# TorchIO-project/torchio

Hardware: NVIDIA H100
Metric: augmented voxels/sec on 256^3 fp32 Compose pipeline (higher is better)
Workload: dtype f32

## Files before the change

include/tio_b200.h:

```cpp
#ifndef TIO_B200_H
#define TIO_B200_H

#include <stddef.h>
#include <stdint.h>

#ifdef __cplusplus
extern "C" {
#endif

#define TIO_ABI_VERSION 2

enum tio_dtype {
  TIO_F32 = 0,
  TIO_U8 = 1,
  TIO_I8 = 2,
  TIO_I16 = 3,
  TIO_I32 = 4,
  TIO_I64 = 5,
  TIO_F16 = 6,
  TIO_BF16 = 7,
  TIO_F64 = 8
};

enum tio_interp { TIO_NEAREST = 0, TIO_LINEAR = 1, TIO_LABEL_PV = 2 };
#define TIO_EXACT_COORDS 0x100

#define TIO_FLAG_PASSTHROUGH 1u
#define TIO_FLAG_ELASTIC 2u

const char* tio_last_error(void);
int tio_abi_version(void);
uint64_t tio_launch_count(void);

size_t tio_resample_workspace_bytes(int B, int OI, int OJ, int OK);

int tio_bspline_prefilter(const void* src, int dtype, float* coeff, const uint8_t* flags,
                          int B, int C, int I, int J, int K, int order, void* stream);
int tio_bspline_resample(const float* coeff, const void* src, void* dst, int dtype,
                         int B, int C, int I, int J, int K,
                         int OI, int OJ, int OK,
                         const float* mat, const float* cp, const uint8_t* flags,
                         int ni, int nj, int nk,
                         const float* spacing_in, const float* spacing_out,
                         int affine_first, int order, void* stream);
int tio_resample(const void* src, void* dst, int dtype,
                 int B, int C, int I, int J, int K,
                 int OI, int OJ, int OK,
                 const float* mat, const float* cp, const uint8_t* flags,
                 int ni, int nj, int nk,
                 const float* spacing_in, const float* spacing_out,
                 int affine_first, int mode, const float* fill, int box_hint,
                 void* workspace, size_t workspace_bytes, void* stream);

int tio_onehot(const void* src, int dtype, int B, int64_t vox, const void* labels, int n,
               float* dst, void* stream);
int tio_label_argmax(const float* sampled, int B, int n, int64_t vox, const void* labels,
                     float pad_label, void* dst, int dtype, void* stream);

int tio_crop_patches(const void* src, void* dst, int elem_bytes, int C, int I, int J, int K,
                     int n, const int32_t* corners, int pi, int pj, int pk, void* stream);

int tio_remap(const void* src, void* dst, int elem_bytes, int B, int C, int I, int J, int K,
              int OI, int OJ, int OK, int off_i, int off_j, int off_k, int mode,
              const void* fill, const uint8_t* flip, void* stream);

int tio_permute(const void* src, void* dst, int elem_bytes, int B, int C, int I, int J, int K,
                int perm0, int perm1, int perm2, int flip_bits, void* stream);

int tio_upload(const void* host_pinned, void* dst_device, size_t bytes, void* stream);

int tio_min_sample0(const float* src, int C, int64_t n, float* fill, void* stream);

int tio_blur(const float* src, float* dst, float* scratch,
             int B, int C, int I, int J, int K,
             const float* taps, const int32_t* radius, int R, int axes_mask,
             const uint8_t* identity, void* stream);

size_t tio_mt19937_table_bytes(void);
int tio_mt19937_build_table(void* host_blob, size_t bytes);
size_t tio_randn_mt19937_workspace_bytes(uint64_t offset, uint64_t n);
int tio_randn_mt19937(uint64_t seed, uint64_t offset, uint64_t n, float* z,
                      const void* table, void* workspace, size_t workspace_bytes,
                      void* stream);

int tio_moments(const float* src, const uint8_t* mask, int64_t n, double* out3, void* stream);
// ... 113 lines not shown
```

torchio_b200/csrc/resample.cu:

```cuda
#include "resample_common.cuh"

namespace tio {

template <typename T, int MODE, bool HAS_CP, bool HAS_FILL>
__global__ void __launch_bounds__(TK* TJ)
resample_kernel(const ResampleArgs a) {
  extern __shared__ float smem_cp[];
  const int tiles_i = (a.OI + TI - 1) / TI;
  const int b = blockIdx.z / tiles_i;
  const int oi0 = (blockIdx.z % tiles_i) * TI;
  const int ok = blockIdx.x * TK + threadIdx.x;
  const int oj = blockIdx.y * TJ + threadIdx.y;
  const int64_t n_in = (int64_t)a.I * a.J * a.K;
  const int64_t n_out = (int64_t)a.OI * a.OJ * a.OK;
  const uint8_t fl = a.flags ? a.flags[b] : 0;
  const T* __restrict__ src = (const T*)a.src + (int64_t)b * a.C * n_in;
  T* __restrict__ dst = (T*)a.dst + (int64_t)b * a.C * n_out;
  const int oi_end = min(oi0 + TI, a.OI);

  if (fl & TIO_FLAG_PASSTHROUGH) {
    if (ok < a.OK && oj < a.OJ)
      for (int c = 0; c < a.C; ++c)
        for (int oi = oi0; oi < oi_end; ++oi) {
          int64_t o = ((int64_t)oi * a.OJ + oj) * a.OK + ok;
// ... 80 lines not shown
  int c = blockIdx.x * blockDim.x + threadIdx.x;
  if (c < C) fill[c] = __int_as_float(0x7f800000);
}

template <bool VEC>
__global__ void __launch_bounds__(256) min_kernel(const float* __restrict__ src, int64_t n,
                                                  float* fill) {
  const int c = blockIdx.y;
  const float* base = src + (int64_t)c * n;
  float m = __int_as_float(0x7f800000);
  const int64_t stride = (int64_t)gridDim.x * blockDim.x;
  const int64_t t0 = (int64_t)blockIdx.x * blockDim.x + threadIdx.x;
  if (VEC) {
    const float4* p = (const float4*)base;
    for (int64_t t = t0; t < (n >> 2); t += stride) {
      float4 v = __ldg(p + t);
      m = fminf(fminf(m, v.x), fminf(v.y, fminf(v.z, v.w)));
    }
  } else {
    for (int64_t t = t0; t < n; t += stride) m = fminf(m, __ldg(base + t));
  }
#pragma unroll
  for (int s = 16; s > 0; s >>= 1) m = fminf(m, __shfl_xor_sync(0xffffffffu, m, s));
  __shared__ float part[8];
  if ((threadIdx.x & 31) == 0) part[threadIdx.x >> 5] = m;
  __syncthreads();
  if (threadIdx.x == 0) {
    for (int t = 1; t < 8; ++t) m = fminf(m, part[t]);
    atomic_min_float(fill + c, m);
  }
}

int launch_resample_tile(const ResampleArgs& a, int dtype, int mode, bool exact_coords, int box_hint,
                         void* workspace, size_t workspace_bytes, cudaStream_t st);
size_t resample_tile_workspace_bytes(int B, int OI, int OJ, int OK);

}

extern "C" int tio_resample(const void* src, void* dst, int dtype, int B, int C, int I, int J,
                            int K, int OI, int OJ, int OK, const float* mat, const float* cp,
                            const uint8_t* flags, int ni, int nj, int nk,
                            const float* spacing_in, const float* spacing_out,
                            int affine_first, int mode, const float* fill, int box_hint,
                            void* workspace, size_t workspace_bytes, void* stream) {
  using namespace tio;
  TIO_CHECK_ARG(src && dst && mat, "tio_resample: null src/dst/mat");
  TIO_CHECK_ARG(src != dst, "tio_resample: src and dst must not alias");
  TIO_CHECK_ARG(B > 0 && C > 0 && I > 0 && J > 0 && K > 0 && OI > 0 && OJ > 0 && OK > 0,
                "tio_resample: non-positive shape");
  const bool exact_coords = (mode & TIO_EXACT_COORDS) != 0;
  mode &= ~TIO_EXACT_COORDS;
  TIO_CHECK_ARG(mode == TIO_NEAREST || mode == TIO_LINEAR || mode == TIO_LABEL_PV, "tio_resample: bad mode %d", mode);
  TIO_CHECK_ARG(mode != TIO_LABEL_PV || (C == 1 && fill),
                "tio_resample: TIO_LABEL_PV needs C == 1 and fill[0] = the pad label");
  TIO_CHECK_ARG(spacing_in && spacing_out, "tio_resample: null spacing");
  TIO_CHECK_ARG(!cp || (ni >= 2 && nj >= 2 && nk >= 2), "tio_resample: control grid < 2 per axis");
  TIO_CHECK_ARG((int64_t)B * ((OI + TI - 1) / TI) <= 65535 && (OJ + TJ - 1) / TJ <= 65535,
                "tio_resample: grid too large (B*ceil(OI/16) and ceil(OJ/4) must be <= 65535)");
  ResampleArgs a;
  a.src = src; a.dst = dst; a.mat = mat; a.cp = cp; a.flags = flags; a.fill = fill;
  a.B = B; a.C = C; a.I = I; a.J = J; a.K = K; a.OI = OI; a.OJ = OJ; a.OK = OK;
  a.ni = ni; a.nj = nj; a.nk = nk;
  auto scale = [](int n_in, int n_out) {
    if (n_in == n_out) return 1.0f;
    return n_out > 1 ? (float)(n_in - 1) / (float)(n_out - 1) : 0.0f;
  };
  a.sc_i = cp ? scale(ni, OI) : 0.f; a.sc_j = cp ? scale(nj, OJ) : 0.f; a.sc_k = cp ? scale(nk, OK) : 0.f;
  const int dims[3] = {I, J, K};
  for (int t = 0; t < 3; ++t) {
    a.sp_in[t] = spacing_in[t]; a.sp_out[t] = spacing_out[t];
    a.nm1[t] = (float)(dims[t] - 1 > 1 ? dims[t] - 1 : 1);
    a.sm1[t] = (float)(dims[t] - 1);
  }
  a.affine_first = affine_first;
  a.cp_in_smem = cp && ((size_t)ni * nj * nk * 12 <= 96 * 1024);
  cudaStream_t st = (cudaStream_t)stream;
  if (box_hint >= 0) {
    const int rc = launch_resample_tile(a, dtype, mode, exact_coords, box_hint, workspace, workspace_bytes, st);
    if (rc == 0) {
      TIO_CHECK_LAUNCH();
      return 0;
    }
    TIO_CHECK_ARG(rc == 1, "tio_resample: TMA tile path failed (code %d)", rc);
  }
  switch (dtype) {
    case TIO_F32: launch_typed<float>(a, mode, st); break;
    case TIO_U8: launch_typed<uint8_t>(a, mode, st); break;
    case TIO_I8: launch_typed<int8_t>(a, mode, st); break;
    case TIO_I16: launch_typed<int16_t>(a, mode, st); break;
    case TIO_I32: launch_typed<int32_t>(a, mode, st); break;
    case TIO_I64: launch_typed<int64_t>(a, mode, st); break;
    default: TIO_CHECK_ARG(false, "tio_resample: unknown dtype %d", dtype);
  }
  TIO_CHECK_LAUNCH();
  return 0;
}

extern "C" size_t tio_resample_workspace_bytes(int B, int OI, int OJ, int OK) {
  return tio::resample_tile_workspace_bytes(B, OI, OJ, OK);
}

extern "C" int tio_min_sample0(const float* src, int C, int64_t n, float* fill, void* stream) {
  using namespace tio;
  TIO_CHECK_ARG(src && fill && C > 0 && n > 0, "tio_min_sample0: bad arguments");
  cudaStream_t st = (cudaStream_t)stream;
  min_init_kernel<<<(C + 31) / 32, 32, 0, st>>>(fill, C);
  launched();
  const bool vec = (((uintptr_t)src & 15) == 0) && ((n & 3) == 0);
  int64_t work = vec ? (n >> 2) : n;
  int blocks = (int)((work + 255) / 256);
  if (blocks > num_sms() * 8) blocks = num_sms() * 8;
  if (blocks < 1) blocks = 1;
  if (vec)
    min_kernel<true><<<dim3(blocks, C), 256, 0, st>>>(src, n, fill);
  else
    min_kernel<false><<<dim3(blocks, C), 256, 0, st>>>(src, n, fill);
  launched();
  TIO_CHECK_LAUNCH();
  return 0;
}
```

torchio_b200/csrc/resample_common.cuh:

```cuda
#pragma once
#include "common.cuh"

namespace tio {


template <typename T>
struct ElemTraits;
template <>
struct ElemTraits<float> {
  static __device__ __forceinline__ float to_f32(float v) { return v; }
  static __device__ __forceinline__ float from_f32(float v) { return v; }
};
#define TIO_INT_TRAITS(T)                                                    \
  template <>                                                                \
  struct ElemTraits<T> {                                                     \
    static __device__ __forceinline__ float to_f32(T v) { return (float)v; } \
    static __device__ __forceinline__ T from_f32(float v) {                  \
      return (T)(long long)v;                \
    }                                                                        \
  };
TIO_INT_TRAITS(uint8_t)
TIO_INT_TRAITS(int8_t)
TIO_INT_TRAITS(int16_t)
TIO_INT_TRAITS(int32_t)
TIO_INT_TRAITS(int64_t)

struct ResampleArgs {
  const void* src;
  void* dst;
  const float* mat;
  const float* cp;
  const uint8_t* flags;
  const float* fill;
  int B, C, I, J, K, OI, OJ, OK;
  int ni, nj, nk;
  float sc_i, sc_j, sc_k;
  float sp_in[3], sp_out[3];
  float nm1[3];
  float sm1[3];
  int affine_first;
  int cp_in_smem;
};

constexpr int TK = 64;
constexpr int TJ = 4;
constexpr int TI = 16;

__device__ __forceinline__ float affine_row(const float* m, float pi, float pj, float pk) {
  float acc = __fmul_rn(pi, m[0]);
  acc = __fmaf_rn(pj, m[1], acc);
  acc = __fmaf_rn(pk, m[2], acc);
  acc = __fmaf_rn(1.0f, m[3], acc);
  return acc;
}

__device__ __forceinline__ float renormalise(float q, float nm1, float sm1) {
  float g = __fsub_rn(__fdiv_rn(__fmul_rn(2.0f, q), nm1), 1.0f);
  return __fmul_rn(__fmul_rn(__fadd_rn(g, 1.0f), 0.5f), sm1);
}


template <typename T>
__device__ __forceinline__ T label_pv_pick(const T tap[8], const float w[8], const unsigned active, const T pad) {
  if (active == 0u) return pad;
  {
    T first = tap[7];
// ... 206 lines not shown
```

torchio_b200/csrc/resample_fast.cu:

```cuda
#include <type_traits>

#include "resample_tile.cuh"

namespace tio {

template <int BOX, int LK>
__device__ __forceinline__ void lane_column(int tid, int& jrow, int& kcol) {
  const int warp = tid >> 5, lane = tid & 31;
  if (LK == 16) {
    constexpr int DJ = (BOX == 20) ? 2 : 4;
    const int half = lane >> 4;
    jrow = (warp % DJ) + (warp / DJ) * (2 * DJ) + half * DJ;
    kcol = lane & 15;
  } else if (LK == 8) {
    jrow = (warp >> 1) * 4 + (lane >> 3);
    kcol = (warp & 1) * 8 + (lane & 7);
  } else {
    jrow = (warp >> 2) * 8 + (lane >> 2);
    kcol = (warp & 3) * 4 + (lane & 3);
  }
}

template <bool HAS_CP, bool HAS_FILL>
__device__ __forceinline__ void exact_planes(const ResampleArgs& a, const TileArgs& ta, int b, bool elastic,
// ... 122 lines not shown
      unpack2(sub2(bc(tz[2 * ax + 1]), u[ax]), qa, qb);
      ma *= __saturatef(fminf(pa, qa));
      mb *= __saturatef(fminf(pb, qb));
    }
    if (!(ma > 0.5f)) va = fill_c;
    if (!(mb > 0.5f)) vb = fill_c;
    unc_a = fabsf(ma - 0.5f) < 1.0e-3f;
    unc_b = fabsf(mb - 0.5f) < 1.0e-3f;
  }
}

template <int BOX, bool HAS_CP, bool HAS_FILL>
__global__ void __launch_bounds__(256, BOX <= 22 ? 4 : 3)
resample_fast_kernel(const __grid_constant__ CUtensorMap tmap, const __grid_constant__ CUtensorMap tmap_s,
                     const __grid_constant__ ResampleArgs a, const __grid_constant__ TileArgs ta,
                     const int4* __restrict__ records) {
  constexpr int BK = box_k_extent(BOX, 4);
  constexpr int NBOX = BOX * BOX * BK;
  constexpr int BOXBYTES = (NBOX * 4 + 15) / 16 * 16;
  constexpr int C1 = BOX * BK, C2 = BK;
  constexpr bool DUAL = HAS_CP && BOX > kSmallBox;
  constexpr int BKS = box_k_extent(kSmallBox, 4);
  constexpr int NBOXS = kSmallBox * kSmallBox * BKS, C1S = kSmallBox * BKS, C2S = BKS;
  extern __shared__ __align__(128) unsigned char smem_raw[];
  float* aux = reinterpret_cast<float*>(smem_raw + BOXBYTES);
  const uint32_t box_u32 = smem_u32(smem_raw);
  const uint32_t bar = smem_u32(aux + 128);
  float* tbase = aux + 132;
  int* cell_tab = reinterpret_cast<int*>(aux + 136);
  unsigned* chg_mask = reinterpret_cast<unsigned*>(aux + 152);

  const int tid = threadIdx.x;
  const int tiles_i = ta.tiles_i;
  const int b = tiles_i == 1 ? (int)blockIdx.z : (int)__umulhi(blockIdx.z, ta.inv_tiles_i);
  const int ti = blockIdx.z - b * tiles_i;
  const int i0 = ti * XT, j0 = blockIdx.y * XT, k0 = blockIdx.x * XT;
  const unsigned tile_id = (blockIdx.z * gridDim.y + blockIdx.y) * gridDim.x + blockIdx.x;
  const int4 rec = __ldg(records + tile_id);
  if ((rec.w & (255 | 2048)) != (1 | 2048)) {
    slow_tile<HAS_CP, HAS_FILL>(a, ta, rec, b, i0, j0, k0);
    return;
  }
  const bool small = DUAL && (rec.w & 4096);
  if (tid == 0) {
    mbar_init(bar, 1);
    mbar_fence_init();
    mbar_expect_tx(bar, (uint32_t)((small ? NBOXS : NBOX) * 4));
    tma_load_4d(box_u32, small ? &tmap_s : &tmap, rec.z, rec.y, rec.x, b * a.C, bar);
  }
  const bool elastic = HAS_CP && (rec.w & 1024);
  const bool masked = HAS_FILL && !(rec.w & 256);
  const float* __restrict__ mp = a.mat + b * 12;
  if (tid >= 32 && tid < 35) {
    const int ax = tid - 32;
    const double t = (double)mp[4 * ax] * i0 + (double)mp[4 * ax + 1] * j0 + (double)mp[4 * ax + 2] * k0 +
                     (double)mp[4 * ax + 3] - (double)(ax == 0 ? rec.x : (ax == 1 ? rec.y : rec.z));
    tbase[ax] = (float)t;
  }
  if (HAS_CP && elastic && tid >= 64 && tid < 96) {
    const int lane = tid - 64;
    auto cell_of = [&](int rel) { return min((int)floorf(__fmul_rn(a.sc_i, (float)(i0 + rel))), a.ni - 1); };
    if (lane < XT) cell_tab[lane] = cell_of(lane);
    bool chg = false;
    if (lane < XT / 2)
      chg = lane == 0 || cell_of(2 * lane) != cell_of(2 * lane - 2) || cell_of(2 * lane + 1) != cell_of(2 * lane - 1);
    const unsigned mask = __ballot_sync(0xffffffffu, chg);
    if (lane == 0) *chg_mask = mask;
  }
// ... 206 lines not shown
```

torchio_b200/csrc/resample_tile.cu:

```cuda
#include <cuda.h>

#include <map>
#include <mutex>

#include "resample_tile.cuh"

namespace tio {

template <int BOX, typename T, int MODE, bool HAS_CP, bool CHECK, bool FASTDIV, int EMODE>
__device__ __forceinline__ void walk_column(
    const ResampleArgs& a, const TileArgs& ta, const T* __restrict__ box,
    const float* __restrict__ cps, const LiEntry* __restrict__ li_tab,
    const LiPair* __restrict__ li_pairs, const float m[12],
    const bool elastic, const bool identity, const uint32_t kbase, const int i0, const int i1,
    const int oj, const int ok, const float fill_c, T* __restrict__ out, const int64_t ostride) {
  constexpr int BK = box_k_extent(BOX, (int)sizeof(T));
  constexpr int C1 = BOX * BK, C2 = BK;
  constexpr int ESH = sizeof(T) == 1 ? 0 : (sizeof(T) == 2 ? 1 : 2);
  const float hd0 = ta.hd[0], hd1 = ta.hd[1], hd2 = ta.hd[2];
  const float rc0 = ta.rcp[0], rc1 = ta.rcp[1], rc2 = ta.rcp[2];
  const float hs0 = ta.hs[0], hs1 = ta.hs[1], hs2 = ta.hs[2];
  const float pj = (float)oj, pk = (float)ok;
  LerpAxis lj, lk;
  int o00 = 0, o01 = 0, o10 = 0, o11 = 0;
// ... 511 lines not shown
                          const TileArgs& ta, dim3 grid,
                          size_t smem, const int4* records, cudaStream_t st);

template <typename T>
static void launch_nearest(int box, const CUtensorMap& tm, const ResampleArgs& a, const TileArgs& ta,
                           dim3 grid, size_t smem, const int4* records, cudaStream_t st) {
  if (box == 24) {
    if (a.cp) launch_tile<24, T, TIO_NEAREST, true, true>(tm, a, ta, grid, smem, records, st);
    else launch_tile<24, T, TIO_NEAREST, false, true>(tm, a, ta, grid, smem, records, st);
  } else {
    if (a.cp) launch_tile<32, T, TIO_NEAREST, true, true>(tm, a, ta, grid, smem, records, st);
    else launch_tile<32, T, TIO_NEAREST, false, true>(tm, a, ta, grid, smem, records, st);
  }
}

template <typename T>
static void launch_label_pv(int box, const CUtensorMap& tm, const ResampleArgs& a, const TileArgs& ta,
                            dim3 grid, size_t smem, const int4* records, cudaStream_t st) {
  if (box == 24) {
    if (a.cp) launch_tile<24, T, TIO_LABEL_PV, true, true>(tm, a, ta, grid, smem, records, st);
    else launch_tile<24, T, TIO_LABEL_PV, false, true>(tm, a, ta, grid, smem, records, st);
  } else {
    if (a.cp) launch_tile<32, T, TIO_LABEL_PV, true, true>(tm, a, ta, grid, smem, records, st);
    else launch_tile<32, T, TIO_LABEL_PV, false, true>(tm, a, ta, grid, smem, records, st);
  }
}

size_t resample_tile_workspace_bytes(int B, int OI, int OJ, int OK) {
  const size_t tiles = (size_t)B * ((OI + XT - 1) / XT) * ((OJ + XT - 1) / XT) * ((OK + XT - 1) / XT);
  return tiles * sizeof(int4);
}

int launch_resample_tile(const ResampleArgs& a, int dtype, int mode, bool exact_coords, int box_hint,
                         void* workspace, size_t workspace_bytes, cudaStream_t st) {
  int esize = 0;
  if (mode == TIO_LINEAR) esize = dtype == TIO_F32 ? 4 : 0;
  else esize = dtype == TIO_U8 ? 1 : dtype == TIO_I16 ? 2 : dtype == TIO_I32 ? 4 : 0;
  if (!esize) return 1;
  const int kalign = 16 / esize;
  if (((int64_t)a.K * esize & 15) || ((uintptr_t)a.src & 15)) return 1;
  if ((int64_t)a.B * a.C > (1 << 30)) return 1;
  EncodeTiledFn encode = encode_tiled_fn();
  if (!encode) return 1;
  int box = 24;
  if (box_hint > 0) box = box_hint <= 20 ? 20 : box_hint <= 22 ? 22 : box_hint <= 24 ? 24 : box_hint <= 28 ? 28 : 32;
  if (mode != TIO_LINEAR) box = box <= 24 ? 24 : 32;
  const int tiles_i = (a.OI + XT - 1) / XT;
  if ((int64_t)a.B * tiles_i > 65535 || (a.OJ + XT - 1) / XT > 65535) return 1;

  CUtensorMap tm;
  const cuuint64_t gdim[4] = {(cuuint64_t)a.K, (cuuint64_t)a.J, (cuuint64_t)a.I, (cuuint64_t)a.B * a.C};
  const cuuint64_t gstride[3] = {(cuuint64_t)a.K * esize, (cuuint64_t)a.J * a.K * esize,
                                 (cuuint64_t)a.I * a.J * a.K * esize};
  const int bk = box_k_extent(box, esize);
  const cuuint32_t bdim[4] = {(cuuint32_t)bk, (cuuint32_t)box, (cuuint32_t)box, 1};
  const cuuint32_t estr[4] = {1, 1, 1, 1};
  const CUtensorMapDataType ttype = mode == TIO_LINEAR ? CU_TENSOR_MAP_DATA_TYPE_FLOAT32
                                    : esize == 1 ? CU_TENSOR_MAP_DATA_TYPE_UINT8
                                    : esize == 2 ? CU_TENSOR_MAP_DATA_TYPE_UINT16
                                                 : CU_TENSOR_MAP_DATA_TYPE_INT32;
  CUresult rc = encode(&tm, ttype, 4, const_cast<void*>(a.src), gdim, gstride,
                       bdim, estr, CU_TENSOR_MAP_INTERLEAVE_NONE, CU_TENSOR_MAP_SWIZZLE_NONE,
                       CU_TENSOR_MAP_L2_PROMOTION_L2_128B, CU_TENSOR_MAP_FLOAT_OOB_FILL_NONE);
  if (rc != CUDA_SUCCESS) return 1;

  TileArgs ta;
  const int dims[3] = {a.I, a.J, a.K};
  bool fast = true;
  for (int t = 0; t < 3; ++t) {
    ta.hd[t] = a.nm1[t] * 0.5f;
    ta.rcp[t] = (float)(1.0 / (double)ta.hd[t]);
    ta.hs[t] = a.sm1[t] * 0.5f;
    (void)dims;
    fast = fast && fastdiv_admitted(ta.hd[t], st);
  }
  ta.n_in = (long long)a.I * a.J * a.K;
  ta.n_out = (long long)a.OI * a.OJ * a.OK;
  ta.tiles_i = tiles_i;
  ta.inv_tiles_i = (unsigned)((1ull << 32) / (unsigned)tiles_i) + 1u;
  ta.sp_in_one = (a.sp_in[0] == 1.f && a.sp_in[1] == 1.f && a.sp_in[2] == 1.f);
  ta.sp_out_one = (a.sp_out[0] == 1.f && a.sp_out[1] == 1.f && a.sp_out[2] == 1.f);
  ta.magic_bytes = (unsigned)kMagicBits << 2;
  for (int t = 0; t < 3; ++t) {
    ta.rsp_in[t] = (float)(1.0 / (double)a.sp_in[t]);
    ta.rsp_out[t] = (float)(1.0 / (double)a.sp_out[t]);
  }

  dim3 grid((a.OK + XT - 1) / XT, (a.OJ + XT - 1) / XT, (unsigned)(a.B * tiles_i));
  const int64_t n_tiles = (int64_t)grid.x * grid.y * grid.z;
  if (n_tiles >= (1ll << 31)) return 1;
  if (!workspace || workspace_bytes < (size_t)n_tiles * sizeof(int4) || ((uintptr_t)workspace & 15)) return 1;
  int4* records = (int4*)workspace;
  const unsigned bounds_blocks = (unsigned)((n_tiles + 127) / 128);
  if (mode != TIO_LINEAR && !fast) return 1;
  const bool dual = !exact_coords && mode == TIO_LINEAR && a.cp && box > kSmallBox;
  const int box_s = dual ? kSmallBox : 0, bk_s = dual ? box_k_extent(kSmallBox, 4) : 0;
  CUtensorMap tm_small = tm;
  if (dual) {
    const cuuint32_t bdim_s[4] = {(cuuint32_t)bk_s, (cuuint32_t)box_s, (cuuint32_t)box_s, 1};
    if (encode(&tm_small, ttype, 4, const_cast<void*>(a.src), gdim, gstride, bdim_s, estr,
               CU_TENSOR_MAP_INTERLEAVE_NONE, CU_TENSOR_MAP_SWIZZLE_NONE, CU_TENSOR_MAP_L2_PROMOTION_L2_128B,
               CU_TENSOR_MAP_FLOAT_OOB_FILL_NONE) != CUDA_SUCCESS)
      return 1;
  }
  if (a.cp) tile_bounds_kernel<true><<<bounds_blocks, 128, 0, st>>>(a, box, kalign, bk, box_s, bk_s, records);
  else tile_bounds_kernel<false><<<bounds_blocks, 128, 0, st>>>(a, box, kalign, bk, box_s, bk_s, records);
  launched();
  const size_t smem = ((size_t)box * box * bk * esize + 15) / 16 * 16 + kAuxFloats * sizeof(float);
  if (mode == TIO_LABEL_PV) {
    if (dtype == TIO_U8) launch_label_pv<uint8_t>(box, tm, a, ta, grid, smem, records, st);
    else if (dtype == TIO_I16) launch_label_pv<int16_t>(box, tm, a, ta, grid, smem, records, st);
    else launch_label_pv<int32_t>(box, tm, a, ta, grid, smem, records, st);
    return 0;
  }
  if (mode == TIO_NEAREST) {
    if (dtype == TIO_U8) launch_nearest<uint8_t>(box, tm, a, ta, grid, smem, records, st);
    else if (dtype == TIO_I16) launch_nearest<int16_t>(box, tm, a, ta, grid, smem, records, st);
    else launch_nearest<int32_t>(box, tm, a, ta, grid, smem, records, st);
    return 0;
  }
  if (!exact_coords) {
    launch_resample_fast(box, tm, tm_small, a, ta, grid, smem, records, st);
    return 0;
  }
  if (box == 20) launch_box<20>(tm, a, ta, grid, smem, fast, records, st);
  else if (box == 22) launch_box<22>(tm, a, ta, grid, smem, fast, records, st);
  else if (box == 24) launch_box<24>(tm, a, ta, grid, smem, fast, records, st);
  else if (box == 28) launch_box<28>(tm, a, ta, grid, smem, fast, records, st);
  else launch_box<32>(tm, a, ta, grid, smem, fast, records, st);
  return 0;
}

}
```

torchio_b200/csrc/resample_tile.cuh:

```cuda
#pragma once
#include <cuda.h>

#include "resample_common.cuh"
#include "tma.cuh"

namespace tio {

constexpr int XT = 16;
constexpr int kSmallBox = 18;
__host__ __device__ constexpr int box_k_extent(int box, int elem_bytes) {
  return (box + 16 / elem_bytes + 16 / elem_bytes - 1) / (16 / elem_bytes) * (16 / elem_bytes);
}
constexpr float kMagic = 12582912.0f;
constexpr int kMagicBits = 0x4B400000;

struct TileArgs {
  float hd[3];
  float rcp[3];
  float hs[3];
  int sp_in_one, sp_out_one;
  float rsp_in[3], rsp_out[3];
  unsigned magic_bytes;
  long long n_in, n_out;
  int tiles_i;
// ... 53 lines not shown
    float b00 = lerp2(lk.l0, p1[o00 + ax], lk.l1, p1[o01 + ax]);
    float b01 = lerp2(lk.l0, p1[o10 + ax], lk.l1, p1[o11 + ax]);
    d[ax] = lerp2(li.l0, lerp2(lj.l0, a00, lj.l1, a01), li.l1, lerp2(lj.l0, b00, lj.l1, b01));
  }
}

__device__ __forceinline__ int axis_points(float scale, int lo, int hi, int* pts) {
  int n = 0;
  pts[n++] = lo;
  if (hi > lo) {
    const float rlo = scale * (float)lo, rhi = scale * (float)hi;
    const int c_first = (int)floorf(rlo) + 1, c_last = (int)ceilf(rhi) - 1;
    for (int c = c_first; c <= c_last; ++c) {
      if (n > 6) return -1;
      const int o = (int)floorf((float)c / scale);
      for (int t = o - 1; t <= o + 1; ++t)
        if (t > lo && t < hi && t > pts[n - 1]) pts[n++] = t;
    }
    pts[n++] = hi;
    if (n > 8) return -1;
  }
  return n;
}

template <bool HAS_CP>
__global__ void __launch_bounds__(128)
tile_bounds_kernel(const ResampleArgs a, const int box, const int kalign, const int bk, const int box_s,
                   const int bk_s, int4* __restrict__ records) {
  const int tiles_i = (a.OI + XT - 1) / XT, tiles_j = (a.OJ + XT - 1) / XT, tiles_k = (a.OK + XT - 1) / XT;
  const int64_t n_tiles = (int64_t)a.B * tiles_i * tiles_j * tiles_k;
  const int64_t tile = (int64_t)blockIdx.x * blockDim.x + threadIdx.x;
  if (tile >= n_tiles) return;
  const unsigned per_b = (unsigned)(tiles_i * tiles_j * tiles_k);
  const int b = (int)(tile / per_b);
  unsigned rest = (unsigned)(tile - (int64_t)b * per_b);
  const int tk = (int)(rest % (unsigned)tiles_k);
  rest /= (unsigned)tiles_k;
  const int tj = (int)(rest % (unsigned)tiles_j), ti = (int)(rest / (unsigned)tiles_j);
  const int i0 = ti * XT, j0 = tj * XT, k0 = tk * XT;
  const int i1 = min(i0 + XT, a.OI) - 1, j1 = min(j0 + XT, a.OJ) - 1, k1 = min(k0 + XT, a.OK) - 1;
  const uint8_t fl = a.flags ? a.flags[b] : 0;
  if (fl & TIO_FLAG_PASSTHROUGH) {
    records[tile] = make_int4(0, 0, 0, 3);
    return;
  }
  const bool elastic = HAS_CP && (fl & TIO_FLAG_ELASTIC);
  float dmn[3] = {0.f, 0.f, 0.f}, dmx[3] = {0.f, 0.f, 0.f};
  bool ok_bounds = true;
  if (elastic) {
    const float* g = a.cp + (int64_t)b * a.ni * a.nj * a.nk * 3;
    int pi[12], pj[12], pk[12];
    const int ni_ = axis_points(a.sc_i, i0, i1, pi);
    const int nj_ = axis_points(a.sc_j, j0, j1, pj);
    const int nk_ = axis_points(a.sc_k, k0, k1, pk);
    if (ni_ < 0 || nj_ < 0 || nk_ < 0) {
      ok_bounds = false;
    } else {
#pragma unroll
      for (int ax = 0; ax < 3; ++ax) { dmn[ax] = 3.0e38f; dmx[ax] = -3.0e38f; }
      for (int qi = 0; qi < ni_; ++qi)
        for (int qj = 0; qj < nj_; ++qj)
          for (int qk = 0; qk < nk_; ++qk) {
            float d[3];
            disp_at(g, a, pi[qi], pj[qj], pk[qk], d);
#pragma unroll
            for (int ax = 0; ax < 3; ++ax) { dmn[ax] = fminf(dmn[ax], d[ax]); dmx[ax] = fmaxf(dmx[ax], d[ax]); }
          }
    }
// ... 105 lines not shown
```

torchio_b200/ops.py:

```python

from __future__ import annotations

import os
import threading

import numpy as np
import torch
from torch import Tensor

from . import _native, tables

DTYPE_CODES = {
    torch.float32: 0, torch.uint8: 1, torch.int8: 2,
    torch.int16: 3, torch.int32: 4, torch.int64: 5,
}
IMAGE_DTYPE_CODES = {**DTYPE_CODES, torch.float16: 6, torch.bfloat16: 7, torch.float64: 8}
NEAREST, LINEAR, LABEL_PV = 0, 1, 2
FLAG_PASSTHROUGH, FLAG_ELASTIC = 1, 2

def launches() -> int:
    return _native.lib().tio_launch_count()


def _launch(name: str, device, *args) -> None:
# ... 96 lines not shown
        dev = torch.empty(offset, dtype=torch.uint8, device=device)
        _launch("tio_upload", dev.device, stage.data_ptr(), dev.data_ptr(), offset)
        _ring.release(slot, torch.device(device))
    else:
        dev = stage.to(device, non_blocking=True)
    out = []
    for s in specs:
        if s is None:
            out.append(None)
            continue
        t, off, nbytes = s
        out.append(dev[off:off + nbytes].view(t.dtype).reshape(t.shape))
    return out


EXACT_COORDS = 0x100
_exact_default = os.environ.get("TIO_B200_EXACT_COORDS", "0") not in ("", "0")


def set_exact_coords(enabled: bool) -> bool:
    global _exact_default
    previous, _exact_default = _exact_default, bool(enabled)
    return previous


def exact_coords_default() -> bool:
    return _exact_default


def resample(
    src: Tensor, mat: Tensor, cp: Tensor | None, flags: Tensor | None,
    spacing_in, spacing_out, *, affine_first: bool, mode: int,
    fill: Tensor | None, out_shape=None, box_hint: int = 0, exact_coords: bool | None = None,
) -> Tensor:
    src = _batch(src, "resample", dtypes=DTYPE_CODES)
    b, c, i, j, k = src.shape
    oi, oj, ok = (i, j, k) if out_shape is None else out_shape
    dst = torch.empty((b, c, oi, oj, ok), dtype=src.dtype, device=src.device)
    ni = nj = nk = 0
    if cp is not None:
        ni, nj, nk = cp.shape[1:4]
    sp_in = np.asarray(spacing_in, dtype=np.float32)
    sp_out = np.asarray(spacing_out, dtype=np.float32)
    workspace, ws_bytes = None, 0
    tiled = (src.dtype == torch.float32 and mode == LINEAR) or (
        mode in (NEAREST, LABEL_PV) and src.dtype in (torch.uint8, torch.int16, torch.int32))
    if box_hint >= 0 and tiled:
        ws_bytes = _native.lib().tio_resample_workspace_bytes(b, oi, oj, ok)
        workspace = torch.empty(ws_bytes, dtype=torch.uint8, device=src.device)
    _launch(
        "tio_resample", src.device, _ptr(src), _ptr(dst), DTYPE_CODES[src.dtype],
        b, c, i, j, k, oi, oj, ok, _ptr(mat), _ptr(cp), _ptr(flags), ni, nj, nk,
        sp_in.ctypes.data, sp_out.ctypes.data, int(bool(affine_first)),
        int(mode) | (EXACT_COORDS if (_exact_default if exact_coords is None else exact_coords) else 0),
        _ptr(fill), int(box_hint), _ptr(workspace), ws_bytes,
    )
    return dst


def bspline_prefilter(src: Tensor, order: int, flags: Tensor | None = None, *, in_place: bool = False) -> Tensor:
    src = _batch(src, "bspline_prefilter", dtypes=DTYPE_CODES, in_place=in_place)
    if in_place and src.dtype != torch.float32:
        raise TypeError(f"bspline_prefilter: in_place needs a float32 tensor, got {src.dtype}")
    coeff = src if in_place else torch.empty(src.shape, dtype=torch.float32, device=src.device)
    _launch("tio_bspline_prefilter", src.device, _ptr(src), DTYPE_CODES[src.dtype], _ptr(coeff), _ptr(flags),
            *src.shape, int(order))
    return coeff


def bspline_resample(
    coeff: Tensor, src: Tensor, mat: Tensor, cp: Tensor | None, flags: Tensor | None,
    spacing_in, spacing_out, *, affine_first: bool, order: int, out_shape=None,
) -> Tensor:
    src = _batch(src, "bspline_resample", dtypes=DTYPE_CODES)
    _check(coeff, "bspline_resample", dtypes=(torch.float32,))
    if coeff.shape != src.shape or not coeff.is_contiguous():
        raise ValueError(f"bspline_resample: coeff must be contiguous of shape {tuple(src.shape)}")
    b, c, i, j, k = src.shape
    oi, oj, ok = (i, j, k) if out_shape is None else out_shape
    dst = torch.empty((b, c, oi, oj, ok), dtype=src.dtype, device=src.device)
    ni = nj = nk = 0
    if cp is not None:
        ni, nj, nk = cp.shape[1:4]
    sp_in = np.asarray(spacing_in, dtype=np.float32)
    sp_out = np.asarray(spacing_out, dtype=np.float32)
    _launch("tio_bspline_resample", src.device, _ptr(coeff), _ptr(src), _ptr(dst), DTYPE_CODES[src.dtype],
            b, c, i, j, k, oi, oj, ok, _ptr(mat), _ptr(cp), _ptr(flags), ni, nj, nk,
            sp_in.ctypes.data, sp_out.ctypes.data, int(bool(affine_first)), int(order))
    return dst
# ... 791 lines not shown
```

torchio_b200/transforms/spatial.py:

```python

from __future__ import annotations

import warnings
from numbers import Number
from pathlib import Path
from typing import Any

import numpy as np
import torch
from torch import Tensor
from torch.distributions import Distribution

from .. import ops, tables
from ..data import AffineMatrix, Image, ImagesBatch, LabelMap, SubjectsBatch
from ..params import Choice, LazyParams, _ParameterRange, to_range, uniform_from_unit
from .base import SpatialTransform, chunk_info

_ORDERS = {
    "nearest": 0, "linear": 1, "quadratic": 2, "cubic": 3,
    "fourth": 4, "fifth": 5, "sixth": 6, "seventh": 7,
}
_NAMES = {v: k for k, v in _ORDERS.items()}
LABEL_INTERPOLATION = "label"
_PAD_MODES = ("minimum", "mean", "otsu")
# ... 711 lines not shown


def _apply_spatial(batch, names, target_space, geometry, *, affine_first, image_interpolation,
                   label_interpolation, antialias, default_pad_value, default_pad_label,
                   one_hot_label_interpolation="linear", max_displacements=None) -> None:
    if not names:
        return
    mats, cps, per_instance = geometry
    first = batch.images[names[0]]
    in_shape, a_in = _shape_of(first), first.affines[0]
    out_shape, a_out = (in_shape, a_in) if target_space is None else target_space
    b = first.batch_size
    packed = tables.spatial_tables(
        mats if per_instance else mats[0], cps if per_instance else cps[0], b,
        a_in.numpy(), a_out.numpy(), per_instance=per_instance,
        has_target=target_space is not None,
    )
    info = chunk_info()
    if info is not None and info.b0 == 0:
        for name in names:
            ib = batch.images[name]
            is_label = issubclass(ib._image_class, LabelMap)
            interp = label_interpolation if is_label else image_interpolation
            if interp == LABEL_INTERPOLATION or _ORDERS[interp] >= 2:
                continue
            native = ib.data if ib.data.dtype in ops.DTYPE_CODES else ib.data.float()
            info.cache[("fill", info.step, name)] = _fill_tensor(native, is_label, default_pad_value,
                                                                 default_pad_label)
    if packed is None:
        return
    if info is None:
        _folding_warning(cps, max_displacements, out_shape, a_out)
    device = first.data.device
    mat_d, cp_d, flags_d = ops.upload(device, packed.mat, packed.cp, packed.flags)
    box_hint = _box_hint(packed, a_in.spacing, a_out.spacing, out_shape)
    target_shape = None if target_space is None else out_shape

    def spline(tensor, order, in_place, source=None):
        coeff = ops.bspline_prefilter(tensor, order, flags_d, in_place=in_place)
        return ops.bspline_resample(
            coeff, tensor if source is None else source, mat_d, cp_d, flags_d, a_in.spacing, a_out.spacing,
            affine_first=affine_first, order=order, out_shape=target_shape)

    keep_original = set(packed.passthrough)
    for name in names:
        ib = batch.images[name]
        is_label = issubclass(ib._image_class, LabelMap)
        interp = label_interpolation if is_label else image_interpolation
        data = ib.data
        if is_label and interp == LABEL_INTERPOLATION:
            def run(tensor, mode, fill, exact):
                return ops.resample(
                    tensor, mat_d, cp_d, flags_d, a_in.spacing, a_out.spacing, affine_first=affine_first,
                    mode=mode, fill=fill, out_shape=target_shape, box_hint=box_hint, exact_coords=exact)
            ib.data = _resample_label_pv(
                data, run, spline, antialias=antialias, a_in=a_in, a_out=a_out,
                one_hot_interpolation=one_hot_label_interpolation, pad_label=default_pad_label)
            ib.affines[:] = [ib.affines[i] if i in keep_original else a_out.clone() for i in range(b)]
            continue
        native = data if data.dtype in ops.DTYPE_CODES else data.float()
        order = _ORDERS[interp]
        if order >= 2:
            smoothed = _antialias(native, a_in, a_out) if antialias and not is_label else native
            out = spline(smoothed, order, False, native)
            out = out if out.dtype == data.dtype else out.to(data.dtype)
            if keep_original and data.dtype not in ops.DTYPE_CODES:
                rows = torch.tensor(sorted(keep_original), device=device)
                out[rows] = data[rows]
            ib.data = out
            ib.affines[:] = [ib.affines[i] if i in keep_original else a_out.clone() for i in range(b)]
            continue
        if info is None:
            fill = _fill_tensor(native, is_label, default_pad_value, default_pad_label)
        else:
            fill = info.cache[("fill", info.step, name)]
        if antialias and not is_label:
            native = _antialias(native, a_in, a_out)
        out = ops.resample(
            native, mat_d, cp_d, flags_d, a_in.spacing, a_out.spacing,
            affine_first=affine_first, mode=ops.NEAREST if interp == "nearest" else ops.LINEAR,
            fill=fill, out_shape=target_shape,
            box_hint=box_hint,
        )
        ib.data = out if out.dtype == data.dtype else out.to(data.dtype)
        ib.affines[:] = [
            ib.affines[i] if i in keep_original else a_out.clone() for i in range(b)
        ]


def _box_hint(packed, sp_in, sp_out, out_shape) -> int:
    m = np.abs(packed.mat.reshape(-1, 3, 4)[:, :, :3])
    extent = (m.sum(axis=2) * 15.0).max(axis=0) + 2.0
    if packed.cp is not None:
        cp = packed.cp
        spacing = np.minimum(np.asarray(sp_in, dtype=np.float64), np.asarray(sp_out))
        variation = np.zeros(3)
        delta = 2.0 * np.abs(cp).reshape(-1, 3).max(axis=0)
        for axis in range(3):
            n_cp, n_out = cp.shape[1 + axis], out_shape[axis]
            if n_cp > 1 and n_out > 1:
                variation += delta * ((n_cp - 1) / (n_out - 1)) * 15.0
        extent = extent + variation / spacing / 3.0
    worst = float(np.max(extent))
    for edge in (20, 22, 24, 28):
        if worst <= edge:
            return edge
    return 32


class Resample(Spatial):

    def __init__(self, target=1, image_interpolation="linear", label_interpolation="nearest",
                 one_hot_label_interpolation="linear", antialias: bool = False, **kwargs: Any) -> None:
        super().__init__(target=target, image_interpolation=image_interpolation,
                         label_interpolation=label_interpolation,
                         one_hot_label_interpolation=one_hot_label_interpolation, antialias=antialias, **kwargs)


class Affine(Spatial):

    def __init__(self, *, scales=1.0, degrees=0.0, translation=0.0, isotropic: bool = False,
                 center: str = "image", default_pad_value="minimum", default_pad_label=0,
                 image_interpolation="linear", label_interpolation="nearest",
                 one_hot_label_interpolation="linear", **kwargs: Any) -> None:
        super().__init__(
            scales=scales, degrees=degrees, translation=translation, isotropic=isotropic,
            center=center, default_pad_value=default_pad_value,
            default_pad_label=default_pad_label, image_interpolation=image_interpolation,
            label_interpolation=label_interpolation,
            one_hot_label_interpolation=one_hot_label_interpolation, **kwargs,
        )
        self._warn_if_noop(
            is_noop=self.scales.is_constant(1.0) and self.degrees.is_constant(0.0)
            and self.translation.is_constant(0.0),
            hint="degrees=(-15, 15)",
        )


class ElasticDeformation(Spatial):

    def __init__(self, *, control_points=None, num_control_points=7, max_displacement=7.5,
                 locked_borders: int = 2, image_interpolation="linear",
# ... 9 lines not shown
```

Baseline: 52.26 billion.

## Group batch elements by per-element TMA box size and launch tiered resample passes

For affine-only fp32 linear resampling, the host now computes the smallest TMA box edge each batch element needs from its own matrix, sorts the elements by edge and launches one bounds+resample pass per edge group. Kernels map a slot index to the real batch element through an element list. The aim is to stop every element loading the batch-wide worst-case box, cutting shared memory per block and TMA traffic for elements with mild transforms. The cost is extra kernel launches, extra tensor-map encodes, an extra upload, and a per-element lookup in the kernels.

```diff
diff --git a/include/tio_b200.h b/include/tio_b200.h
--- a/include/tio_b200.h
+++ b/include/tio_b200.h
@@ -51,6 +51,15 @@
                  const float* spacing_in, const float* spacing_out,
                  int affine_first, int mode, const float* fill, int box_hint,
                  void* workspace, size_t workspace_bytes, void* stream);
+int tio_resample_tiered(const void* src, void* dst, int dtype,
+                        int B, int C, int I, int J, int K,
+                        int OI, int OJ, int OK,
+                        const float* mat, const float* cp, const uint8_t* flags,
+                        int ni, int nj, int nk,
+                        const float* spacing_in, const float* spacing_out,
+                        int affine_first, int mode, const float* fill, int box_hint,
+                        const int* elems, const int* runs, int n_runs,
+                        void* workspace, size_t workspace_bytes, void* stream);
 
 int tio_onehot(const void* src, int dtype, int B, int64_t vox, const void* labels, int n,
                float* dst, void* stream);
diff --git a/torchio_b200/csrc/resample.cu b/torchio_b200/csrc/resample.cu
--- a/torchio_b200/csrc/resample.cu
+++ b/torchio_b200/csrc/resample.cu
@@ -136,17 +136,18 @@
 }
 
 int launch_resample_tile(const ResampleArgs& a, int dtype, int mode, bool exact_coords, int box_hint,
-                         void* workspace, size_t workspace_bytes, cudaStream_t st);
+                         const int* runs, int n_runs, void* workspace, size_t workspace_bytes, cudaStream_t st);
 size_t resample_tile_workspace_bytes(int B, int OI, int OJ, int OK);
 
 }
 
-extern "C" int tio_resample(const void* src, void* dst, int dtype, int B, int C, int I, int J,
-                            int K, int OI, int OJ, int OK, const float* mat, const float* cp,
-                            const uint8_t* flags, int ni, int nj, int nk,
-                            const float* spacing_in, const float* spacing_out,
-                            int affine_first, int mode, const float* fill, int box_hint,
-                            void* workspace, size_t workspace_bytes, void* stream) {
+namespace {
+
+int resample(const void* src, void* dst, int dtype, int B, int C, int I, int J, int K, int OI, int OJ, int OK,
+             const float* mat, const float* cp, const uint8_t* flags, int ni, int nj, int nk,
+             const float* spacing_in, const float* spacing_out, int affine_first, int mode, const float* fill,
+             int box_hint, const int* elems, const int* runs, int n_runs, void* workspace, size_t workspace_bytes,
+             void* stream) {
   using namespace tio;
   TIO_CHECK_ARG(src && dst && mat, "tio_resample: null src/dst/mat");
   TIO_CHECK_ARG(src != dst, "tio_resample: src and dst must not alias");
@@ -162,7 +163,7 @@
   TIO_CHECK_ARG((int64_t)B * ((OI + TI - 1) / TI) <= 65535 && (OJ + TJ - 1) / TJ <= 65535,
                 "tio_resample: grid too large (B*ceil(OI/16) and ceil(OJ/4) must be <= 65535)");
   ResampleArgs a;
-  a.src = src; a.dst = dst; a.mat = mat; a.cp = cp; a.flags = flags; a.fill = fill;
+  a.src = src; a.dst = dst; a.mat = mat; a.cp = cp; a.flags = flags; a.fill = fill; a.elems = elems;
   a.B = B; a.C = C; a.I = I; a.J = J; a.K = K; a.OI = OI; a.OJ = OJ; a.OK = OK;
   a.ni = ni; a.nj = nj; a.nk = nk;
   auto scale = [](int n_in, int n_out) {
@@ -180,7 +181,8 @@
   a.cp_in_smem = cp && ((size_t)ni * nj * nk * 12 <= 96 * 1024);
   cudaStream_t st = (cudaStream_t)stream;
   if (box_hint >= 0) {
-    const int rc = launch_resample_tile(a, dtype, mode, exact_coords, box_hint, workspace, workspace_bytes, st);
+    const int rc = launch_resample_tile(a, dtype, mode, exact_coords, box_hint, runs, n_runs, workspace,
+                                        workspace_bytes, st);
     if (rc == 0) {
       TIO_CHECK_LAUNCH();
       return 0;
@@ -198,6 +200,45 @@
   }
   TIO_CHECK_LAUNCH();
   return 0;
+}
+
+}
+
+extern "C" int tio_resample(const void* src, void* dst, int dtype, int B, int C, int I, int J,
+                            int K, int OI, int OJ, int OK, const float* mat, const float* cp,
+                            const uint8_t* flags, int ni, int nj, int nk,
+                            const float* spacing_in, const float* spacing_out,
+                            int affine_first, int mode, const float* fill, int box_hint,
+                            void* workspace, size_t workspace_bytes, void* stream) {
+  return resample(src, dst, dtype, B, C, I, J, K, OI, OJ, OK, mat, cp, flags, ni, nj, nk, spacing_in, spacing_out,
+                  affine_first, mode, fill, box_hint, nullptr, nullptr, 0, workspace, workspace_bytes, stream);
+}
+
+extern "C" int tio_resample_tiered(const void* src, void* dst, int dtype, int B, int C, int I, int J,
+                                   int K, int OI, int OJ, int OK, const float* mat, const float* cp,
+                                   const uint8_t* flags, int ni, int nj, int nk,
+                                   const float* spacing_in, const float* spacing_out,
+                                   int affine_first, int mode, const float* fill, int box_hint,
+                                   const int* elems, const int* runs, int n_runs,
+                                   void* workspace, size_t workspace_bytes, void* stream) {
+  using namespace tio;
+  TIO_CHECK_ARG(elems && runs && n_runs >= 1 && n_runs <= 5, "tio_resample_tiered: null elems/runs or n_runs %d",
+                n_runs);
+  TIO_CHECK_ARG(dtype == TIO_F32 && mode == TIO_LINEAR && box_hint >= 0 && workspace,
+                "tio_resample_tiered: needs an fp32 image, TIO_LINEAR without TIO_EXACT_COORDS, box_hint >= 0 and"
+                " a workspace");
+  int total = 0, last = 0;
+  for (int r = 0; r < n_runs; ++r) {
+    const int count = runs[2 * r], edge = runs[2 * r + 1];
+    TIO_CHECK_ARG(count > 0 && edge > last && (edge == 20 || edge == 22 || edge == 24 || edge == 28 || edge == 32),
+                  "tio_resample_tiered: run %d: %d elements at edge %d (edges 20/22/24/28/32, ascending)", r, count,
+                  edge);
+    total += count;
+    last = edge;
+  }
+  TIO_CHECK_ARG(total == B, "tio_resample_tiered: the runs hold %d elements, the batch %d", total, B);
+  return resample(src, dst, dtype, B, C, I, J, K, OI, OJ, OK, mat, cp, flags, ni, nj, nk, spacing_in, spacing_out,
+                  affine_first, mode, fill, box_hint, elems, runs, n_runs, workspace, workspace_bytes, stream);
 }
 
 extern "C" size_t tio_resample_workspace_bytes(int B, int OI, int OJ, int OK) {
diff --git a/torchio_b200/csrc/resample_common.cuh b/torchio_b200/csrc/resample_common.cuh
--- a/torchio_b200/csrc/resample_common.cuh
+++ b/torchio_b200/csrc/resample_common.cuh
@@ -32,6 +32,7 @@
   const float* cp;
   const uint8_t* flags;
   const float* fill;
+  const int* elems;
   int B, C, I, J, K, OI, OJ, OK;
   int ni, nj, nk;
   float sc_i, sc_j, sc_k;
diff --git a/torchio_b200/csrc/resample_fast.cu b/torchio_b200/csrc/resample_fast.cu
--- a/torchio_b200/csrc/resample_fast.cu
+++ b/torchio_b200/csrc/resample_fast.cu
@@ -178,8 +178,9 @@
 
   const int tid = threadIdx.x;
   const int tiles_i = ta.tiles_i;
-  const int b = tiles_i == 1 ? (int)blockIdx.z : (int)__umulhi(blockIdx.z, ta.inv_tiles_i);
-  const int ti = blockIdx.z - b * tiles_i;
+  const int slot = tiles_i == 1 ? (int)blockIdx.z : (int)__umulhi(blockIdx.z, ta.inv_tiles_i);
+  const int ti = blockIdx.z - slot * tiles_i;
+  const int b = a.elems ? __ldg(a.elems + slot) : slot;
   const int i0 = ti * XT, j0 = blockIdx.y * XT, k0 = blockIdx.x * XT;
   const unsigned tile_id = (blockIdx.z * gridDim.y + blockIdx.y) * gridDim.x + blockIdx.x;
   const int4 rec = __ldg(records + tile_id);
diff --git a/torchio_b200/csrc/resample_tile.cu b/torchio_b200/csrc/resample_tile.cu
--- a/torchio_b200/csrc/resample_tile.cu
+++ b/torchio_b200/csrc/resample_tile.cu
@@ -567,7 +567,7 @@
 }
 
 int launch_resample_tile(const ResampleArgs& a, int dtype, int mode, bool exact_coords, int box_hint,
-                         void* workspace, size_t workspace_bytes, cudaStream_t st) {
+                         const int* runs, int n_runs, void* workspace, size_t workspace_bytes, cudaStream_t st) {
   int esize = 0;
   if (mode == TIO_LINEAR) esize = dtype == TIO_F32 ? 4 : 0;
   else esize = dtype == TIO_U8 ? 1 : dtype == TIO_I16 ? 2 : dtype == TIO_I32 ? 4 : 0;
@@ -583,30 +583,27 @@
   const int tiles_i = (a.OI + XT - 1) / XT;
   if ((int64_t)a.B * tiles_i > 65535 || (a.OJ + XT - 1) / XT > 65535) return 1;
 
-  CUtensorMap tm;
   const cuuint64_t gdim[4] = {(cuuint64_t)a.K, (cuuint64_t)a.J, (cuuint64_t)a.I, (cuuint64_t)a.B * a.C};
   const cuuint64_t gstride[3] = {(cuuint64_t)a.K * esize, (cuuint64_t)a.J * a.K * esize,
                                  (cuuint64_t)a.I * a.J * a.K * esize};
-  const int bk = box_k_extent(box, esize);
-  const cuuint32_t bdim[4] = {(cuuint32_t)bk, (cuuint32_t)box, (cuuint32_t)box, 1};
   const cuuint32_t estr[4] = {1, 1, 1, 1};
   const CUtensorMapDataType ttype = mode == TIO_LINEAR ? CU_TENSOR_MAP_DATA_TYPE_FLOAT32
                                     : esize == 1 ? CU_TENSOR_MAP_DATA_TYPE_UINT8
                                     : esize == 2 ? CU_TENSOR_MAP_DATA_TYPE_UINT16
                                                  : CU_TENSOR_MAP_DATA_TYPE_INT32;
-  CUresult rc = encode(&tm, ttype, 4, const_cast<void*>(a.src), gdim, gstride,
-                       bdim, estr, CU_TENSOR_MAP_INTERLEAVE_NONE, CU_TENSOR_MAP_SWIZZLE_NONE,
-                       CU_TENSOR_MAP_L2_PROMOTION_L2_128B, CU_TENSOR_MAP_FLOAT_OOB_FILL_NONE);
-  if (rc != CUDA_SUCCESS) return 1;
+  auto encode_box = [&](CUtensorMap* tm, int edge) {
+    const cuuint32_t bdim[4] = {(cuuint32_t)box_k_extent(edge, esize), (cuuint32_t)edge, (cuuint32_t)edge, 1};
+    return encode(tm, ttype, 4, const_cast<void*>(a.src), gdim, gstride, bdim, estr, CU_TENSOR_MAP_INTERLEAVE_NONE,
+                  CU_TENSOR_MAP_SWIZZLE_NONE, CU_TENSOR_MAP_L2_PROMOTION_L2_128B,
+                  CU_TENSOR_MAP_FLOAT_OOB_FILL_NONE) == CUDA_SUCCESS;
+  };
 
   TileArgs ta;
-  const int dims[3] = {a.I, a.J, a.K};
   bool fast = true;
   for (int t = 0; t < 3; ++t) {
     ta.hd[t] = a.nm1[t] * 0.5f;
     ta.rcp[t] = (float)(1.0 / (double)ta.hd[t]);
     ta.hs[t] = a.sm1[t] * 0.5f;
-    (void)dims;
     fast = fast && fastdiv_admitted(ta.hd[t], st);
   }
   ta.n_in = (long long)a.I * a.J * a.K;
@@ -621,48 +618,53 @@
     ta.rsp_out[t] = (float)(1.0 / (double)a.sp_out[t]);
   }
 
-  dim3 grid((a.OK + XT - 1) / XT, (a.OJ + XT - 1) / XT, (unsigned)(a.B * tiles_i));
-  const int64_t n_tiles = (int64_t)grid.x * grid.y * grid.z;
+  const int64_t tiles_per_elem = (int64_t)tiles_i * ((a.OJ + XT - 1) / XT) * ((a.OK + XT - 1) / XT);
+  const int64_t n_tiles = (int64_t)a.B * tiles_per_elem;
   if (n_tiles >= (1ll << 31)) return 1;
   if (!workspace || workspace_bytes < (size_t)n_tiles * sizeof(int4) || ((uintptr_t)workspace & 15)) return 1;
-  int4* records = (int4*)workspace;
-  const unsigned bounds_blocks = (unsigned)((n_tiles + 127) / 128);
   if (mode != TIO_LINEAR && !fast) return 1;
-  const bool dual = !exact_coords && mode == TIO_LINEAR && a.cp && box > kSmallBox;
-  const int box_s = dual ? kSmallBox : 0, bk_s = dual ? box_k_extent(kSmallBox, 4) : 0;
-  CUtensorMap tm_small = tm;
-  if (dual) {
-    const cuuint32_t bdim_s[4] = {(cuuint32_t)bk_s, (cuuint32_t)box_s, (cuuint32_t)box_s, 1};
-    if (encode(&tm_small, ttype, 4, const_cast<void*>(a.src), gdim, gstride, bdim_s, estr,
-               CU_TENSOR_MAP_INTERLEAVE_NONE, CU_TENSOR_MAP_SWIZZLE_NONE, CU_TENSOR_MAP_L2_PROMOTION_L2_128B,
-               CU_TENSOR_MAP_FLOAT_OOB_FILL_NONE) != CUDA_SUCCESS)
-      return 1;
-  }
-  if (a.cp) tile_bounds_kernel<true><<<bounds_blocks, 128, 0, st>>>(a, box, kalign, bk, box_s, bk_s, records);
-  else tile_bounds_kernel<false><<<bounds_blocks, 128, 0, st>>>(a, box, kalign, bk, box_s, bk_s, records);
-  launched();
-  const size_t smem = ((size_t)box * box * bk * esize + 15) / 16 * 16 + kAuxFloats * sizeof(float);
-  if (mode == TIO_LABEL_PV) {
-    if (dtype == TIO_U8) launch_label_pv<uint8_t>(box, tm, a, ta, grid, smem, records, st);
-    else if (dtype == TIO_I16) launch_label_pv<int16_t>(box, tm, a, ta, grid, smem, records, st);
-    else launch_label_pv<int32_t>(box, tm, a, ta, grid, smem, records, st);
-    return 0;
-  }
-  if (mode == TIO_NEAREST) {
-    if (dtype == TIO_U8) launch_nearest<uint8_t>(box, tm, a, ta, grid, smem, records, st);
-    else if (dtype == TIO_I16) launch_nearest<int16_t>(box, tm, a, ta, grid, smem, records, st);
-    else launch_nearest<int32_t>(box, tm, a, ta, grid, smem, records, st);
-    return 0;
-  }
-  if (!exact_coords) {
-    launch_resample_fast(box, tm, tm_small, a, ta, grid, smem, records, st);
-    return 0;
-  }
-  if (box == 20) launch_box<20>(tm, a, ta, grid, smem, fast, records, st);
-  else if (box == 22) launch_box<22>(tm, a, ta, grid, smem, fast, records, st);
-  else if (box == 24) launch_box<24>(tm, a, ta, grid, smem, fast, records, st);
-  else if (box == 28) launch_box<28>(tm, a, ta, grid, smem, fast, records, st);
-  else launch_box<32>(tm, a, ta, grid, smem, fast, records, st);
+  const bool dual = !exact_coords && mode == TIO_LINEAR && a.cp;
+  CUtensorMap tm_small;
+  if (dual && !encode_box(&tm_small, kSmallBox)) return 1;
+
+  const int whole[2] = {a.B, box};
+  if (!a.elems) { runs = whole; n_runs = 1; }
+  CUtensorMap tms[5];
+  for (int r = 0; r < n_runs; ++r)
+    if (!encode_box(&tms[r], runs[2 * r + 1])) return 1;
+  int offset = 0;
+  for (int r = 0; r < n_runs; ++r) {
+    const int count = runs[2 * r], edge = runs[2 * r + 1];
+    const CUtensorMap& tm = tms[r];
+    ResampleArgs ar = a;
+    ar.B = count;
+    ar.elems = a.elems ? a.elems + offset : nullptr;
+    int4* records = (int4*)workspace + offset * tiles_per_elem;
+    offset += count;
+    const dim3 grid((a.OK + XT - 1) / XT, (a.OJ + XT - 1) / XT, (unsigned)(count * tiles_i));
+    const int bk = box_k_extent(edge, esize);
+    const int box_s = dual ? kSmallBox : 0, bk_s = dual ? box_k_extent(kSmallBox, 4) : 0;
+    const unsigned bounds_blocks = (unsigned)((count * tiles_per_elem + 127) / 128);
+    if (ar.cp) tile_bounds_kernel<true><<<bounds_blocks, 128, 0, st>>>(ar, edge, kalign, bk, box_s, bk_s, records);
+    else tile_bounds_kernel<false><<<bounds_blocks, 128, 0, st>>>(ar, edge, kalign, bk, box_s, bk_s, records);
+    launched();
+    const size_t smem = ((size_t)edge * edge * bk * esize + 15) / 16 * 16 + kAuxFloats * sizeof(float);
+    if (mode == TIO_LABEL_PV) {
+      if (dtype == TIO_U8) launch_label_pv<uint8_t>(edge, tm, ar, ta, grid, smem, records, st);
+      else if (dtype == TIO_I16) launch_label_pv<int16_t>(edge, tm, ar, ta, grid, smem, records, st);
+      else launch_label_pv<int32_t>(edge, tm, ar, ta, grid, smem, records, st);
+    } else if (mode == TIO_NEAREST) {
+      if (dtype == TIO_U8) launch_nearest<uint8_t>(edge, tm, ar, ta, grid, smem, records, st);
+      else if (dtype == TIO_I16) launch_nearest<int16_t>(edge, tm, ar, ta, grid, smem, records, st);
+      else launch_nearest<int32_t>(edge, tm, ar, ta, grid, smem, records, st);
+    } else if (!exact_coords) {
+      launch_resample_fast(edge, tm, dual ? tm_small : tm, ar, ta, grid, smem, records, st);
+    } else if (edge == 20) launch_box<20>(tm, ar, ta, grid, smem, fast, records, st);
+    else if (edge == 22) launch_box<22>(tm, ar, ta, grid, smem, fast, records, st);
+    else if (edge == 24) launch_box<24>(tm, ar, ta, grid, smem, fast, records, st);
+    else if (edge == 28) launch_box<28>(tm, ar, ta, grid, smem, fast, records, st);
+    else launch_box<32>(tm, ar, ta, grid, smem, fast, records, st);
+  }
   return 0;
 }
 
diff --git a/torchio_b200/csrc/resample_tile.cuh b/torchio_b200/csrc/resample_tile.cuh
--- a/torchio_b200/csrc/resample_tile.cuh
+++ b/torchio_b200/csrc/resample_tile.cuh
@@ -109,8 +109,9 @@
   const int64_t tile = (int64_t)blockIdx.x * blockDim.x + threadIdx.x;
   if (tile >= n_tiles) return;
   const unsigned per_b = (unsigned)(tiles_i * tiles_j * tiles_k);
-  const int b = (int)(tile / per_b);
-  unsigned rest = (unsigned)(tile - (int64_t)b * per_b);
+  const int slot = (int)(tile / per_b);
+  const int b = a.elems ? a.elems[slot] : slot;
+  unsigned rest = (unsigned)(tile - (int64_t)slot * per_b);
   const int tk = (int)(rest % (unsigned)tiles_k);
   rest /= (unsigned)tiles_k;
   const int tj = (int)(rest % (unsigned)tiles_j), ti = (int)(rest / (unsigned)tiles_j);
diff --git a/torchio_b200/ops.py b/torchio_b200/ops.py
--- a/torchio_b200/ops.py
+++ b/torchio_b200/ops.py
@@ -152,8 +152,10 @@
     src: Tensor, mat: Tensor, cp: Tensor | None, flags: Tensor | None,
     spacing_in, spacing_out, *, affine_first: bool, mode: int,
     fill: Tensor | None, out_shape=None, box_hint: int = 0, exact_coords: bool | None = None,
+    tiers=None,
 ) -> Tensor:
     src = _batch(src, "resample", dtypes=DTYPE_CODES)
+    exact = _exact_default if exact_coords is None else exact_coords
     b, c, i, j, k = src.shape
     oi, oj, ok = (i, j, k) if out_shape is None else out_shape
     dst = torch.empty((b, c, oi, oj, ok), dtype=src.dtype, device=src.device)
@@ -168,13 +170,19 @@
     if box_hint >= 0 and tiled:
         ws_bytes = _native.lib().tio_resample_workspace_bytes(b, oi, oj, ok)
         workspace = torch.empty(ws_bytes, dtype=torch.uint8, device=src.device)
-    _launch(
-        "tio_resample", src.device, _ptr(src), _ptr(dst), DTYPE_CODES[src.dtype],
-        b, c, i, j, k, oi, oj, ok, _ptr(mat), _ptr(cp), _ptr(flags), ni, nj, nk,
-        sp_in.ctypes.data, sp_out.ctypes.data, int(bool(affine_first)),
-        int(mode) | (EXACT_COORDS if (_exact_default if exact_coords is None else exact_coords) else 0),
-        _ptr(fill), int(box_hint), _ptr(workspace), ws_bytes,
-    )
+    args = (_ptr(src), _ptr(dst), DTYPE_CODES[src.dtype],
+            b, c, i, j, k, oi, oj, ok, _ptr(mat), _ptr(cp), _ptr(flags), ni, nj, nk,
+            sp_in.ctypes.data, sp_out.ctypes.data, int(bool(affine_first)),
+            int(mode) | (EXACT_COORDS if exact else 0), _ptr(fill), int(box_hint))
+    if tiers is None:
+        _launch("tio_resample", src.device, *args, _ptr(workspace), ws_bytes)
+        return dst
+    elems, runs = tiers
+    if elems.dtype != torch.int32 or elems.shape != (b,) or not elems.is_cuda:
+        raise ValueError(f"resample: tiers needs an int32 ({b},) cuda element list")
+    runs = np.asarray(runs, dtype=np.int32).reshape(-1, 2)
+    _launch("tio_resample_tiered", src.device, *args, _ptr(elems), runs.ctypes.data, len(runs),
+            _ptr(workspace), ws_bytes)
     return dst
 
 
diff --git a/torchio_b200/transforms/spatial.py b/torchio_b200/transforms/spatial.py
--- a/torchio_b200/transforms/spatial.py
+++ b/torchio_b200/transforms/spatial.py
@@ -767,8 +767,10 @@
     if info is None:
         _folding_warning(cps, max_displacements, out_shape, a_out)
     device = first.data.device
-    mat_d, cp_d, flags_d = ops.upload(device, packed.mat, packed.cp, packed.flags)
     box_hint = _box_hint(packed, a_in.spacing, a_out.spacing, out_shape)
+    order, runs = _box_tiers(packed, box_hint, out_shape)
+    mat_d, cp_d, flags_d, order_d = ops.upload(device, packed.mat, packed.cp, packed.flags, order)
+    tiers = None if order is None else (order_d, runs)
     target_shape = None if target_space is None else out_shape
 
     def spline(tensor, order, in_place, source=None):
@@ -811,11 +813,12 @@
             fill = info.cache[("fill", info.step, name)]
         if antialias and not is_label:
             native = _antialias(native, a_in, a_out)
+        mode = ops.NEAREST if interp == "nearest" else ops.LINEAR
+        tiered = mode == ops.LINEAR and native.dtype == torch.float32 and not ops.exact_coords_default()
         out = ops.resample(
             native, mat_d, cp_d, flags_d, a_in.spacing, a_out.spacing,
-            affine_first=affine_first, mode=ops.NEAREST if interp == "nearest" else ops.LINEAR,
-            fill=fill, out_shape=target_shape,
-            box_hint=box_hint,
+            affine_first=affine_first, mode=mode, fill=fill, out_shape=target_shape,
+            box_hint=box_hint, tiers=tiers if tiered else None,
         )
         ib.data = out if out.dtype == data.dtype else out.to(data.dtype)
         ib.affines[:] = [
@@ -843,6 +846,37 @@
     return 32
 
 
+_BOX_EDGES = (20, 22, 24, 28, 32)
+
+
+def _box_tiers(packed, cap: int, out_shape):
+    if packed.cp is not None:
+        return None, None
+    edges = _affine_box_edges(packed.mat, cap, out_shape)
+    if (edges == cap).all():
+        return None, None
+    order = np.argsort(edges, kind="stable").astype(np.int32)
+    values, counts = np.unique(edges, return_counts=True)
+    return order, [(int(n), int(e)) for e, n in zip(values, counts)]
+
+
+def _affine_box_edges(mat, cap: int, out_shape) -> np.ndarray:
+    m = np.asarray(mat, dtype=np.float64).reshape(-1, 3, 4)
+    lin = np.abs(m[:, :, :3])
+    span = np.maximum(np.asarray(out_shape, dtype=np.float64) - 1.0, 0.0)
+    q_max = np.abs(m[:, :, 3]) + lin @ span
+    width = lin.sum(axis=2) * 15.0 + 2.0 * (0.02 + 1e-5 * q_max) + 1e-3
+    with np.errstate(invalid="ignore"):
+        need = np.floor(width) + 3.0
+        need[:, 2] += 3.0
+        need[~np.isfinite(need)] = np.inf
+        edges = np.full(len(m), cap, dtype=np.int32)
+        for edge in reversed([e for e in _BOX_EDGES if e < cap]):
+            fits = (need[:, 0] <= edge) & (need[:, 1] <= edge) & (need[:, 2] <= (edge + 7) // 4 * 4)
+            edges[fits] = edge
+    return edges
+
+
 class Resample(Spatial):
 
     def __init__(self, target=1, image_interpolation="linear", label_interpolation="nearest",
```

Result: faster. 54.55 billion, median of 6 (+4.4%).
